# andvg3/LipVQ-VAE

Hardware: AMD Instinct MI355X
Metric: actions tokenized/sec (encode+quantize) at B=4096 T=128 K=1024, 1/2/4/8 GPU (higher is better)
Workload: dtype f32

## Files before the change

lipvq-vae_amd/csrc/lipvq_fused.hip:

```cpp
#include <string.h>
#include <atomic>

#include "lipvq_mlp.h"
#include "lipvq_screen.h"

#define FUSED_WAVES 8
#define FUSED_THREADS (FUSED_WAVES * 64)
#define FUSED_HIST_MAX 2048
#define LQ_RING8_TC 1
#define LQ_RING8_NB 3
#define LQ_RING13_NB 3
constexpr int fused_ring_tc(int S) { return (S <= 2) ? 4 : (S <= 4) ? 2 : (S == 8) ? LQ_RING8_TC : 1; }
constexpr int fused_ring_nb(int S) { return (S <= 4) ? 4 : (S == 8) ? LQ_RING8_NB : LQ_RING13_NB; }
#define LQ_COARSE_TC_WIDE 2
constexpr int fused_ring_tc_coarse(int S) { return S == 8 ? LQ_COARSE_TC_WIDE * fused_ring_tc(S) : fused_ring_tc(S); }

struct Gelu2 {
    lq_v2f x, t, u, s;
    __device__ __forceinline__ void stage0(float a, float b) {
        x = (lq_v2f){a, b};
        t = x * x;
        u = lq_fma2(t, lq_bc2(0.11111111111111111111f), lq_bc2(-1.0f));
        s = lq_fma2(lq_bc2(0.00012666420661844313f), u, lq_bc2(-0.00043783686123788357f));
        s = lq_fma2(s, u, lq_bc2(0.0008924771682359278f));
// ... 45 lines not shown
template <int S, bool FAST>
__host__ __device__ static bool fused_hist_fits(int A, int K) {
    return K <= FUSED_HIST_MAX && fused_lds_bytes_nohist<S, FAST>(A) + (size_t)K * 4 <= (size_t)160 * 1024;
}
template <int S, bool FAST>
static size_t fused_lds_bytes(int A, int K) {
    return fused_lds_bytes_nohist<S, FAST>(A) + (fused_hist_fits<S, FAST>(A, K) ? (size_t)K * 4 : 0);
}

struct TokArgs {
    const float* x;
    const float* packed;
    const unsigned char* packed16;
    const unsigned char* prep;
    const float* cb;
    int64_t* idx;
    float* zq;
    unsigned long long* usage;
    float* ze_out;
    int* amb_count;
    int* amb_list;
    const float* w2q;
    float* pre0;
    float* pre1;
    float* pre2;
    int64_t N;
    int A, D, K;
    float gamma;
    int coarse;
    int inplace;
    int defer_ze;
    int nt_ze;
    int ze_ring;
};

template <int S, bool FAST, bool TRAIN, int WAVES, bool COARSE = false, bool VQ = false>
__device__ __forceinline__ void tokenize_body(const TokArgs& a) {
    static_assert(!(FAST && TRAIN), "training uses the parity arithmetic");
    static_assert(!VQ || !FAST, "the ReLU instance: parity arithmetic");
    constexpr int THREADS = WAVES * 64;
    constexpr int TCF = COARSE ? fused_ring_tc_coarse(S) : fused_ring_tc(S), NBF = fused_ring_nb(S);
    using RingCfg = ScreenCfg<S, TCF, COARSE>;
    constexpr size_t SLAB_STRIDE = ScreenCfg<S, fused_ring_tc(S), false>::STAGE_BYTES;
    constexpr int T0 = 2, T1 = 4, T2 = (S + 1) / 2;
    constexpr int S1 = 16 * T0, S2 = 16 * T1;
    constexpr bool STREAM2 = !FAST && S >= LQ_STREAM2_MIN_S;
    static_assert(!FAST || (S % 2 == 0 && S <= 8), "fast mode: D in {32, 64, 128}");
    extern __shared__ __attribute__((aligned(16))) unsigned char lds[];
#ifdef LQ_STAMPS
    const long long st_top = __builtin_amdgcn_s_memtime();
    const long long st_top_rt = (long long)__builtin_amdgcn_s_memrealtime();
#endif

    const PackedLayout PL = packed_layout(a.A, 32 * T0, 32 * T1, 16 * S);
    const PrepLayout L = prep_layout(a.K, a.D);
    const int S0 = PL.S0;
    const int S0q = (S0 + 3) / 4;
    const int S0h = (a.A + 15) / 16;
    float* w_P0 = reinterpret_cast<float*>(lds);
    float* w_B0 = w_P0 + (FAST ? T0 * S0h * 256 : T0 * S0q * 256);
    float* w_P1 = w_B0 + 32 * T0;
    float* w_B1 = w_P1 + (FAST ? T1 * (2 * T0) * 256 : T1 * (S1 / 4) * 256);
    float* w_P2 = w_B1 + 32 * T1;
    float* w_B2 = w_P2 + (FAST ? T2 * (2 * T1) * 256 : STREAM2 ? 0 : T2 * (S2 / 4) * 256);
    float* w_mu = w_B2 + 32 * T2;
    unsigned char* stage0 = reinterpret_cast<unsigned char*>(w_mu + 16 * S);
    constexpr size_t RING_OWN = (size_t)NBF * RingCfg::STAGE_BYTES + 1024, RING_FINE = lq_ring_bytes<S, fused_ring_tc(S), NBF>();
    constexpr size_t STAGES_BYTES = RING_OWN > RING_FINE ? RING_OWN : RING_FINE;
    static_assert(STAGES_BYTES >= (size_t)WAVES * LQ_DECIDE_BYTES, "the decision's per-wave transposes live in the stage ring");
    constexpr size_t WSLICE = (STAGES_BYTES >= (size_t)WAVES * 8192) ? 8192 : LQ_DECIDE_BYTES;
    static_assert(LQ_DECIDE_BYTES >= 4096 && WSLICE >= LQ_DECIDE_BYTES, "a slice holds the transposes and four staged KiB");
    unsigned* hist = reinterpret_cast<unsigned*>(stage0 + ((STAGES_BYTES + 63) & ~(size_t)63));
    const bool use_hist = a.usage && fused_hist_fits<S, FAST>(a.A, a.K);

    const int tid = threadIdx.x, lane = tid & 63;
    const int wave = __builtin_amdgcn_readfirstlane(tid >> 6);
    const int ln = lane & 31, h = lane >> 5;

    const unsigned* hdr = reinterpret_cast<const unsigned*>(a.prep);
    const unsigned char* tiles = a.prep + (COARSE ? L.o_tiles_hi : L.o_tiles);
    const size_t tile_bytes = COARSE ? L.tile_bytes_hi : L.tile_bytes;
    const int sz = lq_scale_exp(1.0f + __uint_as_float(hdr[4]));
    const float fz = lq_pow2f(sz);
    const float fown = lq_pow2f(sz + (int)hdr[3]);
    const float tiny2 = (float)(16 * S) * lq_pow2f(-10 - 2 * sz);
    const int64_t nblk = (a.N + WAVES * 32 - 1) / (WAVES * 32);
    constexpr int XPF = 8;
    const bool x_pref = !FAST && a.A <= 2 * XPF;
    float xq[XPF];
    constexpr int LANE_W_MIN_S = 8;
    auto load_x = [&](int64_t blk_, float (&out)[XPF]) {
        int64_t r_ = (blk_ * WAVES + wave) * 32 + ln;
        r_ = r_ < a.N ? r_ : a.N - 1;
        const int64_t last = a.N * a.A - 1;
        int h_x = h;
        if constexpr (S >= LANE_W_MIN_S) asm volatile("" : "+v"(h_x));
#pragma unroll
        for (int q = 0; q < XPF; ++q) {
            const int k = 2 * q + h_x;
            int64_t i_ = r_ * a.A + k;
            i_ = i_ < last ? i_ : last;
            const float v = a.x[i_];
            out[q] = (k < a.A) ? v : 0.0f;
        }
// ... 89 lines not shown
#define LQ_STAMP(i) do { const long long t_ = __builtin_amdgcn_s_memtime(); st_acc[i] += t_ - st_prev; st_prev = t_; } while (0)
#else
#define LQ_STAMP(i) do { } while (0)
#endif
    constexpr bool DEFER_GATHER = !FAST;
    int pend_k = 0;
    bool pend_ok = false;
    int64_t pend_row0 = 0;
    bool have_pend = false;
    int64_t ze_shift = 0;
    auto store_ze_tile = [&](const int64_t row, const int t, const f32x16& acc) {
            {
                float lo8[8], hi8[8];
#pragma unroll
                for (int j = 0; j < 8; ++j) {
                    const auto sw = __builtin_amdgcn_permlane32_swap(__float_as_uint(acc[j]), __float_as_uint(acc[8 + j]), false, false);
                    lo8[j] = __uint_as_float(sw[0]);
                    hi8[j] = __uint_as_float(sw[1]);
                }
                if (row < a.N && 2 * t + h < S) {
                    float4* dst = reinterpret_cast<float4*>(a.ze_out + (size_t)(row - ze_shift) * a.D + 32 * t + 16 * h);
                    typedef float lq_f4v __attribute__((ext_vector_type(4)));
#pragma unroll
                    for (int q = 0; q < 4; ++q)
                        if (S > 4 || TRAIN || a.nt_ze) __builtin_nontemporal_store((lq_f4v){lo8[2 * q], hi8[2 * q], lo8[2 * q + 1], hi8[2 * q + 1]}, reinterpret_cast<lq_f4v*>(dst) + q);
                        else reinterpret_cast<lq_f4v*>(dst)[q] = (lq_f4v){lo8[2 * q], hi8[2 * q], lo8[2 * q + 1], hi8[2 * q + 1]};
                }
            }
    };
    for (int64_t blk = blockIdx.x; blk < nblk; blk += gridDim.x) {
#ifdef LQ_STAMPS
        st_prev = __builtin_amdgcn_s_memtime();
#endif
        ze_shift = a.ze_ring ? (blk - (int64_t)blockIdx.x) * (WAVES * 32) : 0;
        f16x8 ah[S], al[S];
        constexpr bool DEFER_ZE = S <= 4 && !TRAIN;
        f32x16 zdef;
        float row_n2, row_a2, row_fz, row_fown;
      auto encode = [&]() {
        int lane_w = lane;
        if constexpr (S >= LANE_W_MIN_S) asm volatile("" : "+v"(lane_w));
        const int h_w = lane_w >> 5;
        const int64_t row0 = (blk * WAVES + wave) * 32;
        const int64_t row = row0 + ln;
        const int64_t rowc = row < a.N ? row : a.N - 1;
        float n2 = 0.0f, a2lo = 0.0f, amax = 0.0f;
        float zt[VQ ? T2 : 1][16];
        auto finish_tile = [&](const int t, f32x16& acc) {
            if constexpr (TRAIN) lq_tile_store16(a.pre2, a.D, row, row < a.N, t, h, acc, a.D, true);
          if constexpr (VQ) {
#pragma unroll
            for (int r = 0; r < 16; ++r) {
                if (2 * t + (r >> 3) >= S) { zt[t][r] = 0.0f; continue; }
                const float zv = acc[r] > 0.0f ? acc[r] : 0.0f;
                acc[r] = zv;
                const float v = zv - w_mu[32 * t + 2 * r + h_w];
                zt[t][r] = v;
                n2 = lq_fma(v, v, n2);
                amax = fmaxf(amax, lq_abs(v));
            }
          } else {
            if constexpr (!FAST) {
                lq_v2f chk = lq_bc2(0.0f);
#pragma unroll
                for (int r = 0; r < 16; r += 2) chk = lq_nonfinite_acc2((lq_v2f){acc[r], acc[r + 1]}, chk);
                if (__builtin_amdgcn_ballot_w64(!(chk.x == 0.0f && chk.y == 0.0f)) != 0ull) {
#pragma unroll
                    for (int r = 0; r < 16; ++r) acc[r] = lq_sigmoid(acc[r]);
                } else {
#pragma unroll
                    for (int r = 0; r < 16; r += 2) {
                        if (2 * t + (r >> 3) >= S) continue;
                        const lq_v2f z2 = lq_sigmoid2_finite((lq_v2f){acc[r], acc[r + 1]});
                        acc[r] = z2.x; acc[r + 1] = z2.y;
                    }
                }
            }
#pragma unroll
            for (int r = 0; r < 16; ++r) {
                if (2 * t + (r >> 3) >= S) continue;
                const float zv = FAST ? __builtin_amdgcn_rcpf(1.0f + __builtin_amdgcn_exp2f(acc[r] * -1.44269504088896341f)) : acc[r];
                acc[r] = zv;
                const float v = zv - w_mu[32 * t + 2 * r + h_w];
                n2 = lq_fma(v, v, n2);
                const float vs = v * fz;
                const _Float16 vh = (_Float16)vs;
                const float rs = vs - (float)vh;
                ah[2 * t + (r >> 3)][r & 7] = vh;
                al[2 * t + (r >> 3)][r & 7] = (_Float16)rs;
                if constexpr (COARSE) a2lo = lq_fma(rs, rs, a2lo);
            }
          }
            if (a.ze_out) {
                if (DEFER_ZE && a.defer_ze && t == T2 - 1) zdef = acc;
                else store_ze_tile(row, t, acc);
            }
        };

        if constexpr (!FAST) {
            auto gelu_fixup = [&](f32x16& out, const f32x16& pre) {
                float mx = 0.0f;
#pragma unroll
                for (int r = 0; r < 16; r += 2) asm("v_max3_f32 %0, %1, |%2|, |%3|" : "=v"(mx) : "v"(mx), "v"(pre[r]), "v"(pre[r + 1]));
                if (__builtin_amdgcn_ballot_w64(!(mx * mx < 18.0f)) != 0ull) {
#pragma unroll
                    for (int r = 0; r < 16; ++r)
                        if (!(pre[r] * pre[r] < 18.0f)) out[r] = lq_gelu_tail(pre[r]);
                }
            };
            auto bias16 = [&](const float* wb, int t) {
                f32x16 b;
                const float4* p4 = reinterpret_cast<const float4*>(wb + (2 * t + h) * 16);
#pragma unroll
                for (int q = 0; q < 4; ++q) { const float4 v = p4[q]; b[4 * q] = v.x; b[4 * q + 1] = v.y; b[4 * q + 2] = v.z; b[4 * q + 3] = v.w; }
                return b;
            };
            f32x16 h0[T0];
            constexpr int NTRIP = (16 * S + 63) / 64;
            constexpr int GP = (STAGES_BYTES >= (size_t)WAVES * 8192) ? 8 : 4;
            constexpr int NROUND = NTRIP * (8 / GP);
            unsigned char* gstage = stage0 + (size_t)wave * WSLICE;
            const bool gnow = DEFER_GATHER && have_pend && a.zq;
            if (gnow) lq_gather_dma<GP>(gstage, a.cb, pend_k, pend_ok, pend_row0, a.N, a.D, lane, 0, 0);
            {
#pragma unroll
                for (int t = 0; t < T0; ++t) h0[t] = bias16(w_B0, t);
// ... 256 lines not shown
                    if (2 * t + (r >> 3) >= S) continue;
                    const float vs = zt[t][r] * fzr;
                    const _Float16 vh = (_Float16)vs;
                    const float rs = vs - (float)vh;
                    ah[2 * t + (r >> 3)][r & 7] = vh;
                    al[2 * t + (r >> 3)][r & 7] = (_Float16)rs;
                    if constexpr (COARSE) a2lo = lq_fma(rs, rs, a2lo);
                }
        }
        if constexpr (COARSE) a2lo += __shfl_xor(a2lo, 32, 64);
        row_a2 = a2lo;
      };
        encode();
        float frow[16];
        if constexpr (VQ) lq_row_factors(row_fown, lane, frow);
        else {
#pragma unroll
            for (int r = 0; r < 16; ++r) frow[r] = fown;
        }
        float m1[16], m2[16];
        int k1[16];
#pragma unroll
        for (int r = 0; r < 16; ++r) { m1[r] = INFINITY; m2[r] = INFINITY; k1[r] = 0; }
        LQ_STAMP(3);
        if (x_pref) load_x(blk + gridDim.x < nblk ? blk + gridDim.x : blk, xq);
        constexpr bool PACKF = S <= 4 || S > 8 || COARSE;
        const float zn = COARSE ? lq_coarse_zn(row_a2, row_n2, row_fz, row_fown, __uint_as_float(hdr[5])) : 0.0f;
        float znr[16];
        if constexpr (COARSE) lq_row_factors(zn, lane, znr);
        else {
#pragma unroll
            for (int r = 0; r < 16; ++r) znr[r] = 0.0f;
        }
        const bool have_def = DEFER_ZE && a.defer_ze && a.ze_out != nullptr;
        auto deferred_ze = [&]() { store_ze_tile((blk * WAVES + wave) * 32 + ln, T2 - 1, zdef); };
        lq_screen_core<S, THREADS, TCF, NBF, PACKF, COARSE, 4, decltype(deferred_ze)>(ah, al, tiles, L.ntiles, stage0, tid, frow, znr, m1, m2, k1, have_def, deferred_ze);
        LQ_STAMP(4);
        const unsigned keep_mask = PACKF ? ~((1u << lq_pack_bits(L.ntiles)) - 1u) : 0xffffffffu;
        unsigned char* scratch = stage0 + (size_t)wave * WSLICE;
        const int64_t row0 = (blk * WAVES + wave) * 32;
        const int64_t row = row0 + ln;
        int my_k;
        LqDecision dec;
        bool certified = lq_screen_decide<PACKF, COARSE>(m1, m2, k1, scratch, hdr, row_n2, row_fown, a.gamma, a.K, a.D, lane,
                                                         my_k, dec, PACKF ? lq_pow2f(lq_pack_bits(L.ntiles) - 23) : 0.0f, keep_mask,
                                                         zn, tiles, tile_bytes, ScreenCfg<S, TCF, COARSE>::FRAG_BYTES);
        const bool row_sane = VQ || row_n2 >= tiny2;
        certified = certified && row_sane;
        if (!COARSE && a.inplace)
            certified = lq_screen_decide_inplace<PACKF, 2 * S, VQ ? LIPVQ_DIST_SQSUM : LIPVQ_DIST_NORM>(
                dec, certified, row_sane, my_k, row0 - ze_shift, row < a.N, a.amb_count, a.ze_out, a.cb, a.K, lane, keep_mask, scratch);
        else
            lq_screen_emit<PACKF>(dec, certified, row_sane, my_k, row, row < a.N, a.amb_count, a.amb_list, a.N, a.K, lane, keep_mask, scratch);
        if (h == 0 && row < a.N && certified) {
            a.idx[row] = (int64_t)my_k;
            if (use_hist) atomicAdd(&hist[my_k], 1u);
        }
        if (a.usage && !use_hist) lq_usage_add(a.usage, my_k, h == 0 && row < a.N && certified);
        if (DEFER_GATHER) { pend_k = my_k; pend_ok = certified; pend_row0 = row0; }
        else if (a.zq) lq_screen_gather(a.cb, a.zq, my_k, certified, row0, a.N, a.D, lane);
        if (DEFER_GATHER) have_pend = true;
        LQ_STAMP(5);
        LQ_STAMP(6);
    }
    if (DEFER_GATHER && have_pend && a.zq) lq_screen_gather(a.cb, a.zq, pend_k, pend_ok, pend_row0, a.N, a.D, lane);
#ifdef LQ_STAMPS
    if (lane == 0) {
        long long* dbg = LqWorkspace::from_lists(a.amb_list, a.N).stamps() + ((size_t)blockIdx.x * WAVES + wave) * 16;
        for (int i = 0; i < 7; ++i) dbg[i] = st_acc[i];
        dbg[7] = 0;
        dbg[8] = __builtin_amdgcn_s_memtime() - st_begin;
        dbg[9] = st_begin;
        dbg[10] = st_begin - st_top;
        dbg[11] = (long long)__builtin_amdgcn_s_memrealtime();
        dbg[12] = st_top_rt;
    }
#endif
    lq_ws_publish(a.amb_count);
    if (use_hist) {
        for (int i = tid; i < a.K; i += THREADS) {
            const unsigned c = hist[i];
            if (c) atomicAdd(&a.usage[i], (unsigned long long)c);
        }
    }
}

template <int S, bool FAST, bool TRAIN = false, bool COARSE = false, bool VQ = false>
__global__ __launch_bounds__(FUSED_THREADS) void tokenize_kernel(TokArgs a) {
    tokenize_body<S, FAST, TRAIN, FUSED_WAVES, COARSE, VQ>(a);
}
template <int S, bool FAST, bool TRAIN, bool COARSE = false>
__global__ __launch_bounds__(256) __attribute__((amdgpu_waves_per_eu(1, 1))) void tokenize_kernel_w4(TokArgs a) {
    tokenize_body<S, FAST, TRAIN, 4, COARSE>(a);
}

__global__ void mlp3_pack_f16_kernel(const float* __restrict__ W0, const float* __restrict__ W1, const float* __restrict__ W2,
                                     _Float16* __restrict__ out, int A, int J0, int J1, int D) {
    const int S0h = (A + 15) / 16, S1h = J0 / 16, S2h = J1 / 16;
    const int T0 = J0 / 32, T1 = J1 / 32, T2 = (D + 31) / 32;
    const size_t n0 = (size_t)T0 * S0h * 512, n1 = (size_t)T1 * S1h * 512, n2 = (size_t)T2 * S2h * 512;
    size_t g = (size_t)blockIdx.x * blockDim.x + threadIdx.x;
    if (g >= n0 + n1 + n2) return;
    const float* W;
    int K, J, Sh;
    size_t e = g;
    if (e < n0) { W = W0; K = A; J = J0; Sh = S0h; }
    else if (e < n0 + n1) { e -= n0; W = W1; K = J0; J = J1; Sh = S1h; }
    else { e -= n0 + n1; W = W2; K = J1; J = D; Sh = S2h; }
    const int j = (int)(e & 7), lane = (int)((e >> 3) & 63);
    const size_t ts = e >> 9;
    const int s = (int)(ts % Sh), t = (int)(ts / Sh);
    const int f = 32 * t + feat_of_tile_row(lane & 31);
    const int k = 16 * s + 2 * j + (lane >> 5);
    out[g] = (_Float16)((f < J && k < K) ? W[(size_t)f * K + k] : 0.0f);
}

extern "C" size_t lipvq_mlp3_packed_f16_bytes(int A, int J0, int J1, int D) {
    if (A <= 0 || J0 <= 0 || J1 <= 0 || D <= 0 || (J0 & 31) || (J1 & 31)) return 0;
    const size_t S0h = (A + 15) / 16, T2 = (D + 31) / 32;
    return ((size_t)(J0 / 32) * S0h + (size_t)(J1 / 32) * (J0 / 16) + T2 * (J1 / 16)) * 512 * sizeof(_Float16);
}

extern "C" int lipvq_mlp3_pack_f16_f32(const float* W0, const float* W1, const float* W2, void* packed16, int A, int J0,
                                       int J1, int D, void* stream) {
    if (!W0 || !W1 || !W2 || !packed16) return fail(LIPVQ_EINVAL, "mlp3_pack_f16: null pointer");
    const size_t bytes = lipvq_mlp3_packed_f16_bytes(A, J0, J1, D);
// ... 2 lines not shown
    hipLaunchKernelGGL(mlp3_pack_f16_kernel, dim3((unsigned)((n + 255) / 256)), dim3(256), 0, (hipStream_t)stream, W0, W1, W2,
                       (_Float16*)packed16, A, J0, J1, D);
    return check_launch("mlp3_pack_f16");
}

extern "C" int lipvq_tokenize_supported(int A, int J0, int J1, int D, int K) {
    return (A > 0 && A <= 64 && J0 == 64 && J1 == 128 && K > 0 && (D == 32 || D == 64 || D == 128 || D == 208)) ? 1 : 0;
}

extern "C" int lipvq_tokenize_fast_supported(int A, int J0, int J1, int D, int K) {
    return (lipvq_tokenize_supported(A, J0, J1, D, K) && D != 208) ? 1 : 0;
}

#define LQ_DEFAULT_DEFER_ZE 0
struct LqSchedule { int defer_ze, nt_ze; };
static std::atomic<int> g_tuned[64];
static LqSchedule lq_schedule(int ring) {
    LqSchedule sc{LQ_DEFAULT_DEFER_ZE, ring ? 0 : 1};
    int dev = 0;
    if (hipGetDevice(&dev) == hipSuccess && dev >= 0 && dev < 64) {
        const int t = g_tuned[dev].load(std::memory_order_relaxed);
        if (t) { sc.defer_ze = (t - 1) & 1; sc.nt_ze = ((t - 1) >> 1) & 1; }
    }
    if (const char* e = lq_knob("tok_defer_ze")) sc.defer_ze = e[0] != '0';
    if (const char* e = lq_knob("tok_nt_ze")) sc.nt_ze = e[0] != '0';
    return sc;
}

static int lq_inplace(bool have_ze, int coarse, int K) {
    const char* e = lq_knob("tok_inplace");
    return (have_ze && !coarse && K <= LQ_LISTS_ALL_K && !(e && e[0] == '0')) ? 1 : 0;
}
static int lq_ze_ring(bool caller_wants_ze, int inplace) { return (!caller_wants_ze && inplace) ? 1 : 0; }

static int tok_waves(int64_t N) {
    const char* e = lq_knob("tok_shape");
    if (e && !strcmp(e, "w8rg1")) return 8;
    if (e && !strcmp(e, "w4rg1")) return 4;
    return N <= 4 * 32 * 256 ? 4 : 8;
}

__global__ void w2q_pack_kernel(const float* __restrict__ P2, float* __restrict__ out, int T2, int S2) {
    const size_t i = (size_t)blockIdx.x * blockDim.x + threadIdx.x;
    if (i >= (size_t)T2 * (S2 / 4) * 256) return;
    const int q = (int)(i & 3), l = (int)((i >> 2) & 63), sq = (int)((i >> 8) % (S2 / 4)), t = (int)((i >> 8) / (S2 / 4));
    out[i] = P2[((size_t)t * S2 + 4 * sq + q) * 64 + l];
}

template <int S, bool FAST, bool TRAIN, int WAVES, bool COARSE, bool VQ>
static int launch_tokenize_as(const TokArgs& a, hipStream_t st) {
    static_assert(WAVES == 8 || !VQ, "the plain VQVAE's instances have 8 waves");
    static LqLdsReserve reserved;
    const size_t lds = fused_lds_bytes<S, FAST>(a.A, a.K);
    if (lds > 160 * 1024) return fail(LIPVQ_EUNSUPPORTED, "tokenize: %zu B of LDS needed", lds);
    void (*kfn)(TokArgs);
    if constexpr (WAVES == 4) kfn = tokenize_kernel_w4<S, FAST, TRAIN, COARSE>;
    else kfn = tokenize_kernel<S, FAST, TRAIN, COARSE, VQ>;
    if (int rc = lipvq_reserve_lds(reserved, (const void*)kfn, lds, "tokenize")) return rc;
    if (a.w2q) {
        const PackedLayout PL = packed_layout(a.A, 64, 128, a.D);
        const size_t n = LqWorkspace::w2q_floats(a.D);
        hipLaunchKernelGGL(w2q_pack_kernel, dim3((unsigned)((n + 255) / 256)), dim3(256), 0, st, a.packed + PL.oP2,
                           LqWorkspace::from_lists(a.amb_list, a.N).w2q(), PL.T2, PL.S2);
    }
    const int64_t unit = (int64_t)WAVES * 32;
    const int64_t nblk = (a.N + unit - 1) / unit;
    const int64_t cap = 256;
    hipLaunchKernelGGL(kfn, dim3((unsigned)(nblk < cap ? nblk : cap)), dim3(WAVES * 64), lds, st, a);
    return check_launch("tokenize");
}

enum { TOK_TRAIN, TOK_FAST, TOK_PARITY, TOK_VQ };
template <int S, int MODE>
static int launch_tokenize(const TokArgs& a, hipStream_t st) {
    if constexpr (MODE == TOK_TRAIN) {
        return a.coarse ? launch_tokenize_as<S, false, true, 8, true, false>(a, st) : launch_tokenize_as<S, false, true, 8, false, false>(a, st);
    } else if constexpr (MODE == TOK_FAST) {
        if constexpr (S <= 8) return launch_tokenize_as<S, true, false, 8, false, false>(a, st);
        else return LIPVQ_EUNSUPPORTED;
    } else if constexpr (MODE == TOK_PARITY) {
        const int waves = tok_waves(a.N);
        if constexpr (S >= 8) {
            if (a.coarse && waves == 4) return launch_tokenize_as<S, false, false, 4, true, false>(a, st);
        }
        if (a.coarse) return launch_tokenize_as<S, false, false, 8, true, false>(a, st);
        if (waves == 4) return launch_tokenize_as<S, false, false, 4, false, false>(a, st);
        return launch_tokenize_as<S, false, false, 8, false, false>(a, st);
    } else {
        if (a.pre0) return a.coarse ? launch_tokenize_as<S, false, true, 8, true, true>(a, st) : launch_tokenize_as<S, false, true, 8, false, true>(a, st);
        return a.coarse ? launch_tokenize_as<S, false, false, 8, true, true>(a, st) : launch_tokenize_as<S, false, false, 8, false, true>(a, st);
    }
}

extern "C" int lipvq_tokenize_workspace_init(void* workspace, void* stream) {
    if (!workspace) return fail(LIPVQ_EINVAL, "tokenize_workspace_init: null pointer");
    hipError_t e = hipMemsetAsync(workspace, 0, LqWorkspace::kHeaderBytes, (hipStream_t)stream);
    if (e != hipSuccess) return fail(LIPVQ_EHIP, "tokenize_workspace_init: %s", hipGetErrorString(e));
    return LIPVQ_OK;
}

extern "C" size_t lipvq_tokenize_workspace_bytes(int64_t N, int D) { return (N <= 0 || D <= 0) ? 0 : LqWorkspace::tokenize_bytes(N, D); }

static int tokenize_run(const char* who, bool vq, const float* x, const float* packed, const void* packed16, const float* const* raw6,
                        const float* codebook, const void* prep, int64_t* idx, float* zq, int64_t* usage, float* ze_out,
                        float* pre0, float* pre1, float* pre2, void* workspace, int64_t N, int A, int J0, int J1, int D, int K,
                        void* stream) {
    if (N < 0) return fail(LIPVQ_EINVAL, "%s: N < 0", who);
    if (N == 0) return LIPVQ_OK;
    if (!x || !packed || !codebook || !prep || !idx || !workspace || (vq ? !ze_out : !raw6)) return fail(LIPVQ_EINVAL, "%s: null pointer", who);
    for (int i = 0; !vq && i < 6; ++i)
        if (!raw6[i]) return fail(LIPVQ_EINVAL, "%s: raw encoder weight %d is null", who, i);
    if (!lipvq_tokenize_supported(A, J0, J1, D, K))
        return fail(LIPVQ_EUNSUPPORTED, "%s: unsupported shape A=%d J0=%d J1=%d D=%d K=%d", who, A, J0, J1, D, K);
    if (N > 2147483647LL) return fail(LIPVQ_EUNSUPPORTED, "%s: N too large", who);
    if ((((uintptr_t)codebook | (uintptr_t)zq | (uintptr_t)ze_out | (uintptr_t)workspace | (uintptr_t)packed16 | (uintptr_t)pre0 |
          (uintptr_t)pre1 | (uintptr_t)pre2) & 15) != 0)
        return fail(LIPVQ_EINVAL, "%s: codebook, zq, ze_out, workspace, packed16 and pre0..2 must be 16-byte aligned", who);
    if (packed16 && !lipvq_tokenize_fast_supported(A, J0, J1, D, K))
        return fail(LIPVQ_EUNSUPPORTED, "%s: D=%d has no fast instance (32, 64, 128)", who, D);
    hipStream_t st = (hipStream_t)stream;
    const LqWorkspace ws{(unsigned char*)workspace, N, D};
    const LqOut out{idx, zq, usage};
    const int coarse = !packed16 ? lq_screen_coarse(lq_screen_S(D), K) : 0;
    int64_t ze_rows = packed16 ? 131072 : INT64_MAX;
    if (const char* ev = lq_knob("tok_ze_rows")) ze_rows = atoll(ev);
    float* ze_buf = (ze_out || !(coarse || N <= ze_rows)) ? ze_out : ws.ze_scratch();
    TokArgs a{};
    a.x = x;
    a.packed = packed;
    a.packed16 = (const unsigned char*)packed16;
    a.prep = (const unsigned char*)prep;
    a.cb = codebook;
    a.idx = idx;
    a.zq = zq;
    a.usage = (unsigned long long*)usage;
    a.ze_out = ze_buf;
    a.amb_count = ws.live();
    a.amb_list = ws.row_list();
    a.w2q = LqWorkspace::w2q_floats(D) ? ws.w2q() : nullptr;
    a.pre0 = pre0;
    a.pre1 = pre1;
    a.pre2 = pre2;
    a.N = N;
    a.A = A;
    a.D = D;
    a.K = K;
    a.gamma = LIPVQ_SCREEN_GAMMA;
    a.coarse = coarse;
    a.inplace = lq_inplace(ze_buf != nullptr, coarse, K);
    a.ze_ring = lq_ze_ring(ze_out != nullptr, a.inplace);
    const LqSchedule sc = lq_schedule(a.ze_ring);
    a.defer_ze = sc.defer_ze;
    a.nt_ze = sc.nt_ze;
    int rc = LIPVQ_OK;
    lq_dispatch<TOK_TRAIN, TOK_FAST, TOK_PARITY, TOK_VQ>(vq ? TOK_VQ : pre0 ? TOK_TRAIN : packed16 ? TOK_FAST : TOK_PARITY, [&](auto mode) {
        lq_dispatch<32, 64, 128, 208>(D, [&](auto d) { rc = launch_tokenize<(d() + 15) / 16, mode()>(a, st); });
    });
    if (!rc && !a.inplace) {
        if (ze_buf) rc = lipvq_launch_rows(ze_buf, 0, codebook, out, ws, K, st, vq ? LIPVQ_DIST_SQSUM : LIPVQ_DIST_NORM);
        else rc = lipvq_launch_rows_encode(x, raw6, A, codebook, out, ws, K, st);
    }
    if (rc) (void)hipMemsetAsync(ws.header(), 0, LqWorkspace::kHeaderBytes, st);
    return rc;
}

extern "C" int lipvq_tokenize_f32(const float* x, const float* packed, const float* const* raw6, const float* codebook,
                                  const void* prep, int64_t* idx, float* zq, int64_t* usage, float* ze_out,
                                  void* workspace, int64_t N, int A, int J0, int J1, int D, int K, void* stream) {
    return tokenize_run("tokenize", false, x, packed, nullptr, raw6, codebook, prep, idx, zq, usage, ze_out, nullptr, nullptr, nullptr,
                        workspace, N, A, J0, J1, D, K, stream);
}

extern "C" int lipvq_tokenize_tune_f32(const float* x, const float* packed, const float* const* raw6, const float* codebook,
                                       const void* prep, int64_t* idx, float* zq, int64_t* usage, float* ze_out, void* workspace,
                                       int64_t N, int A, int J0, int J1, int D, int K, void* stream, int launches, int* choice,
                                       float* ms4) {
    hipStream_t st = (hipStream_t)stream;
    hipStreamCaptureStatus cs = hipStreamCaptureStatusNone;
    if (hipStreamIsCapturing(st, &cs) == hipSuccess && cs != hipStreamCaptureStatusNone)
        return fail(LIPVQ_EINVAL, "tokenize_tune: the stream is capturing (the tuner synchronises)");
    if (launches < 1) return fail(LIPVQ_EINVAL, "tokenize_tune: launches < 1");
    if (lq_screen_S(D) > 4) {
        if (choice) *choice = -1;
        if (ms4) for (int c = 0; c < 4; ++c) ms4[c] = 0.0f;
        return LIPVQ_OK;
    }
    int dev = 0;
    if (hipGetDevice(&dev) != hipSuccess || dev < 0 || dev >= 64) return fail(LIPVQ_EINVAL, "tokenize_tune: device index");
    hipEvent_t e0, e1;
    if (hipEventCreate(&e0) != hipSuccess || hipEventCreate(&e1) != hipSuccess) return fail(LIPVQ_EHIP, "tokenize_tune: hipEventCreate");
    const int before = g_tuned[dev].load(std::memory_order_relaxed);
    float best[4] = {INFINITY, INFINITY, INFINITY, INFINITY};
    int rc = LIPVQ_OK;
    auto run = [&](int n) {
        for (int i = 0; i < n && !rc; ++i)
            rc = lipvq_tokenize_f32(x, packed, raw6, codebook, prep, idx, zq, usage, ze_out, workspace, N, A, J0, J1, D, K, stream);
    };
    run(launches);
    for (int round = 0; round < 2 && !rc; ++round)
        for (int c = 0; c < 4 && !rc; ++c) {
            g_tuned[dev].store(1 + c, std::memory_order_relaxed);
            run((launches + 1) / 2);
            (void)hipEventRecord(e0, st);
            run(launches);
            (void)hipEventRecord(e1, st);
            if (hipEventSynchronize(e1) != hipSuccess) rc = fail(LIPVQ_EHIP, "tokenize_tune: hipEventSynchronize");
            float ms = 0.0f;
            if (!rc && hipEventElapsedTime(&ms, e0, e1) == hipSuccess && ms / launches < best[c]) best[c] = ms / launches;
        }
    (void)hipEventDestroy(e0);
    (void)hipEventDestroy(e1);
    if (rc) { g_tuned[dev].store(before, std::memory_order_relaxed); return rc; }
    const int ring = lq_ze_ring(ze_out != nullptr, lq_inplace(true, lq_screen_coarse(lq_screen_S(D), K), K));
    const int dflt = LQ_DEFAULT_DEFER_ZE | ((ring ? 0 : 1) << 1);
    int win = dflt;
    for (int c = 0; c < 4; ++c) if (best[c] < 0.995f * best[dflt] && best[c] < best[win]) win = c;
    g_tuned[dev].store(1 + win, std::memory_order_relaxed);
    if (choice) *choice = win;
    if (ms4) for (int c = 0; c < 4; ++c) ms4[c] = best[c];
    return LIPVQ_OK;
}

extern "C" int lipvq_tokenize_train_f32(const float* x, const float* packed, const float* const* raw6, const float* codebook,
                                        const void* prep, int64_t* idx, float* zq, int64_t* usage, float* ze_out, float* pre0,
                                        float* pre1, float* pre2, void* workspace, int64_t N, int A, int J0, int J1, int D, int K,
                                        void* stream) {
    if (!ze_out || !pre0 || !pre1 || !pre2) return fail(LIPVQ_EINVAL, "tokenize_train: z_e and the three pre-activation buffers are required");
    return tokenize_run("tokenize_train", false, x, packed, nullptr, raw6, codebook, prep, idx, zq, usage, ze_out, pre0, pre1, pre2,
                        workspace, N, A, J0, J1, D, K, stream);
}

// ... 24 lines not shown
```

lipvq-vae_amd/csrc/lipvq_screen.h:

```cpp
#ifndef LIPVQ_SCREEN_H_
#define LIPVQ_SCREEN_H_
#include <hip/hip_fp16.h>

#include <type_traits>

#include "lipvq_common.h"

typedef _Float16 f16x8 __attribute__((ext_vector_type(8)));

#define LIPVQ_SCREEN_GAMMA 3.814697265625e-06f
#define SCREEN_WAVES 8

struct PrepLayout {
    int S, Dpad, Kpad, ntiles;
    size_t o_hdr, o_mu, o_tiles, tile_bytes, total;
    size_t o_tiles_hi, tile_bytes_hi;
};

#define LIPVQ_SCREEN_GAMMA_WIDE 1.52587890625e-05f
#define LQ_SCREEN_NARROW_MAX_S 13

__host__ __device__ static inline int lq_screen_S(int D) {
    const int s = (D + 15) / 16;
    return D <= 0 ? 0 : s <= 2 ? 2 : s <= 4 ? 4 : s <= 8 ? 8 : s <= 13 ? 13 : s <= 16 ? 16 : s <= 24 ? 24 : s <= 32 ? 32 : 0;
// ... 78 lines not shown
}

template <int S, bool PACK, bool COARSE = false>
__device__ __forceinline__ void lq_track_after_mfma(int j, const f32x16& acc, float e2, float en, const float (&frow)[16],
                                                    const float (&znr)[16], int id, unsigned keep_mask, float (&m1)[16],
                                                    float (&m2)[16], int (&k1)[16]) {
    constexpr int NM = COARSE ? S : 3 * S;
    const int lo = (16 * j) / NM, hi = (16 * (j + 1)) / NM;
#pragma unroll
    for (int r = 0; r < 16; ++r)
        if (r >= lo && r < hi) {
            const float v = COARSE ? acc[r] : lq_fma(e2, frow[r], acc[r]);
            lq_track_one<PACK>(v, id, keep_mask, m1[r], m2[r], k1[r]);
        }
}

template <int N>
__device__ __forceinline__ void lq_wait_vmcnt() {
    static_assert(N >= 0 && N < 64, "vmcnt immediate");
    asm volatile("s_waitcnt vmcnt(%0)" ::"n"(N) : "memory");
}
template <int S, int TC_, int NB>
constexpr size_t lq_ring_bytes() { return (size_t)NB * ScreenCfg<S, TC_>::STAGE_BYTES + 1024; }

__host__ __device__ static inline int lq_pack_bits(int ntiles) { int b = 1; while ((1 << b) < ntiles) ++b; return b; }

struct LqNoDeferred { __device__ __forceinline__ void operator()() const {} };
template <int S, int NT, int TC_ = screen_default_tc(S), int NB = 4, bool PACK = false, bool COARSE = false, int NDEF = 0,
          typename DEFERRED = LqNoDeferred>
__device__ __forceinline__ void lq_screen_core(const f16x8 (&ah)[S], const f16x8 (&al)[S],
                                               const unsigned char* __restrict__ tiles, int ntiles,
                                               unsigned char* stage0, int tid, const float (&frow)[16], const float (&znr)[16],
                                               float (&m1)[16], float (&m2)[16], int (&k1)[16],
                                               bool have_def = false, DEFERRED deferred = DEFERRED()) {
    using C = ScreenCfg<S, TC_, COARSE>;
    static_assert(NB >= 3 && NB <= 4, "ring of 3 or 4 stage buffers");
    constexpr int NW = NT / 64;
    constexpr int CHUNKS = (C::STAGE_BYTES + 1023) / 1024;
    constexpr int CPW = (CHUNKS + NW - 1) / NW;
    constexpr int PD = NB - 1;
    constexpr int NSTEP = C::TC * S;
    constexpr int MID = (C::TC >= 2) ? (C::TC / 2) * S : S / 2;
    constexpr int FR = 2;
    constexpr int FD = FR - 1;
    constexpr int PERIOD = ((C::TC & 1) || (NSTEP % FR)) ? 2 : 1;
    static_assert(C::STAGE_BYTES >= 1024 && C::STAGE_BYTES % 16 == 0, "stage copies are whole KiB pieces");
    static_assert(NSTEP - FD >= MID, "next-stage fragments are read after the hand-over");
    static_assert(CPW * PD < 64, "vmcnt immediate");
    const int lane = tid & 63, ln = lane & 31;
    const int wave = __builtin_amdgcn_readfirstlane(tid >> 6);
    const int nstage = ntiles / C::TC;
    unsigned char* dummy = stage0 + (size_t)NB * C::STAGE_BYTES;
    typedef __attribute__((address_space(3))) void* lds_ptr_t;
    typedef const __attribute__((address_space(1))) void* glb_ptr_t;
    auto stage_dma = [&](int st, int buf) {
        const bool real = st < nstage;
        const unsigned char* src = tiles + (real ? (size_t)st * C::STAGE_BYTES : (size_t)0);
        unsigned char* dst = stage0 + (size_t)buf * C::STAGE_BYTES;
#pragma unroll
        for (int j = 0; j < CPW; ++j) {
            int chunk = wave + j * NW;
            chunk = chunk < CHUNKS ? chunk : CHUNKS - 1;
            int off = chunk * 1024;
            off = off + 1024 <= C::STAGE_BYTES ? off : C::STAGE_BYTES - 1024;
            unsigned char* d = real ? dst + off : dummy;
            __builtin_amdgcn_global_load_lds((glb_ptr_t)(src + off + lane * 16), (lds_ptr_t)d, 16, 0, 0);
        }
    };
    auto frag = [&](const unsigned char* tb, int s, int hl) {
        return COARSE ? *reinterpret_cast<const f16x8*>(tb + ((size_t)s * 64 + lane) * 16)
                      : *reinterpret_cast<const f16x8*>(tb + (((size_t)s * 2 + hl) * 64 + lane) * 16);
    };
    lq_wg_barrier();
#pragma unroll
    for (int p = 0; p < PD; ++p) stage_dma(p, p);
    static_assert((PD - 1) * CPW + NDEF < 64, "vmcnt immediate");
    if (NDEF > 0 && have_def) {
        deferred();
        lq_wait_vmcnt<(PD - 1) * CPW + NDEF>();
    } else {
        lq_wait_vmcnt<(PD - 1) * CPW>();
    }
    lq_wg_barrier();

    f32x16 accA, accB;
#pragma unroll
    for (int r = 0; r < 16; ++r) accB[r] = INFINITY;
    float e2A = 0.0f, e2B = 0.0f;
    int codeA = 0, codeB = 0;
    const unsigned keep_mask = PACK ? ~((1u << lq_pack_bits(ntiles)) - 1u) : 0xffffffffu;
    f16x8 fh[FR], fl[FR];
    float e2q[2] = {0.0f, 0.0f};
    float enq[2] = {0.0f, 0.0f};
    float enA = 0.0f, enB = 0.0f;
#pragma unroll
    for (int g = 0; g < FD; ++g) {
        fh[g] = frag(stage0, g, 0);
        if constexpr (!COARSE) fl[g] = frag(stage0, g, 1);
    }
    e2q[0] = reinterpret_cast<const float*>(stage0 + C::FRAG_BYTES)[ln];
    if constexpr (COARSE) enq[0] = reinterpret_cast<const float*>(stage0 + C::FRAG_BYTES + 128)[ln];
    static_assert(FD <= S, "prologue reads stay in tile 0");
    int buf = 0;
    auto do_stage = [&](auto POS, int st) {
        constexpr int par = (decltype(POS)::value * C::TC) & 1;
        constexpr int so = (decltype(POS)::value * NSTEP) % FR;
        const unsigned char* sb = stage0 + (size_t)buf * C::STAGE_BYTES;
        int nbuf = buf + 1; nbuf = nbuf == NB ? 0 : nbuf;
        const unsigned char* nsb = stage0 + (size_t)nbuf * C::STAGE_BYTES;
#pragma unroll
        for (int g = 0; g < NSTEP; ++g) {
            const int c = g / S, s = g % S;
            if (g == MID) {
                if (NDEF > 0 && have_def && st == 0) lq_wait_vmcnt<(PD >= 2 ? (PD - 2) * CPW : 0) + (PD >= 2 ? NDEF : 0)>();
                else lq_wait_vmcnt<(PD >= 2 ? (PD - 2) * CPW : 0)>();
                lq_wg_barrier();
                int b = buf + PD; b = b >= NB ? b - NB : b;
                stage_dma(st + PD, b);
            }
            f32x16& acc = (((c + par) & 1) == 0) ? accA : accB;
            const f32x16& prev = (((c + par) & 1) == 0) ? accB : accA;
            const float e2_prev = (((c + par) & 1) == 0) ? e2B : e2A;
            const float en_prev = (((c + par) & 1) == 0) ? enB : enA;
            const int code_prev = (((c + par) & 1) == 0) ? codeB : codeA;
            if (s == 0) {
                const float e2c = e2q[(c + par) & 1];
                const float enc = enq[(c + par) & 1];
#pragma unroll
                for (int r = 0; r < 16; ++r) acc[r] = COARSE ? lq_fma(-znr[r], enc, e2c * frow[r]) : 0.0f;
                int code = PACK ? (st * C::TC + c) : (st * C::TC + c) * 32 + ln;
                if constexpr (PACK) asm volatile("" : "+v"(code));
                if (((c + par) & 1) == 0) { e2A = e2c; enA = enc; codeA = code; } else { e2B = e2c; enB = enc; codeB = code; }
            }
            const f16x8 bh = fh[(g + so) % FR];
            f16x8 bl = bh;
            if constexpr (!COARSE) bl = fl[(g + so) % FR];
            auto read_ahead = [&]() {
                const int g1 = g + FD;
                const unsigned char* base = (g1 < NSTEP) ? sb : nsb;
                const int gg = (g1 < NSTEP) ? g1 : g1 - NSTEP;
                const unsigned char* tb = base + (size_t)(gg / S) * C::TILE_BYTES;
                fh[(g1 + so) % FR] = frag(tb, gg % S, 0);
                if constexpr (!COARSE) fl[(g1 + so) % FR] = frag(tb, gg % S, 1);
                if (gg % S == 0) {
                    e2q[(g1 / S + par) & 1] = reinterpret_cast<const float*>(tb + C::FRAG_BYTES)[ln];
                    if constexpr (COARSE) enq[(g1 / S + par) & 1] = reinterpret_cast<const float*>(tb + C::FRAG_BYTES + 128)[ln];
                }
// ... 326 lines not shown
        if constexpr (DIST == LIPVQ_DIST_NORM) {
            float a = 0.0f;
#pragma unroll
            for (int i = 0; i < DCH; ++i) { const float d = zv[i] - c[8 * i + j]; a = lq_fma(d, d, a); }
            s = __shfl(a, 8 * g, 64);
#pragma unroll
            for (int l = 1; l < 8; ++l) s = s + __shfl(a, 8 * g + l, 64);
            s = lq_sqrt(s);
        } else {
            float acc[4] = {0.f, 0.f, 0.f, 0.f};
#pragma unroll
            for (int i = 0; i < DCH; ++i) {
                const int q = (i < (DCH / 4) * 4) ? (i & 3) : 0;
                const float d = zv[i] - c[8 * i + j];
                acc[q] = acc[q] + d * d;
            }
            const float vl = ((acc[0] + acc[1]) + acc[2]) + acc[3];
            s = __shfl(vl, 8 * g, 64);
#pragma unroll
            for (int l = 1; l < 8; ++l) s = s + __shfl(vl, 8 * g + l, 64);
        }
        const float v = (live && s == s) ? s : INFINITY;
        const int kk = live ? code : 0x7fffffff;
        LQ_TAKE_MIN(best_v, best_k, v, kk);
    }
    LQ_WAVE_MIN(best_v, best_k, 8);
    if (best_k < 0 || best_k >= K) {
        const int fb = scanning ? __builtin_ctz(lm_eff) : LQ_SLOT_FIRST(cl, n0);
        best_k = (fb >= 0 && fb < K) ? fb : 0;
    }
    return best_k;
}

template <bool PACK, int DCH, int DIST>
__device__ __forceinline__ bool lq_screen_decide_inplace(const LqDecision& dec, bool certified, bool lists_ok, int& my_k, int64_t row0,
                                                         bool row_valid, int* __restrict__ amb_count, const float* __restrict__ z,
                                                         const float* __restrict__ cb, int K, int lane, unsigned keep_mask,
                                                         unsigned char* wave_lds) {
    const bool need = row_valid && !certified;
    if (__builtin_amdgcn_ballot_w64(need) == 0ull) return certified;
    const int ln = lane & 31, h = lane >> 5;
    unsigned long long lm = __builtin_amdgcn_ballot_w64(h == 0 && need);
    if (lane == __builtin_ctzll(lm)) (void)lq_ws_reserve(amb_count, __builtin_popcountll(lm));
    int head;
    unsigned mask;
    int codes[LQ_CAND_MAX];
    lq_emit_candidates<PACK>(dec, lists_ok, K, lane, keep_mask, wave_lds, head, mask, codes);
    __builtin_amdgcn_wave_barrier();
    int* parts = reinterpret_cast<int*>(wave_lds);
    static_assert(LQ_CAND_MAX == 6 && 32 * 16 * 4 <= LQ_DECIDE_BYTES, "a part is {n, mask, six codes}");
    if (need) {
        typedef int lq_i4 __attribute__((ext_vector_type(4)));
        lq_i4* out4 = reinterpret_cast<lq_i4*>(parts + ln * 16 + 8 * h);
        out4[0] = lq_i4{head, (int)mask, codes[0], codes[1]};
        out4[1] = lq_i4{codes[2], codes[3], codes[4], codes[5]};
    }
    __builtin_amdgcn_s_waitcnt(0xC07F);
    __builtin_amdgcn_wave_barrier();
    constexpr int D = DCH * 8;
    while (lm) {
        const int r = __builtin_ctzll(lm);
        lm &= lm - 1ull;
        const float* zr = z + (size_t)(row0 + r) * D;
        const int bk = lq_lists_row<DCH, DIST>([&](int f) { return __hip_atomic_load(zr + f, __ATOMIC_RELAXED, __HIP_MEMORY_SCOPE_AGENT); },
                                               cb, K, parts + r * 16, lane, true);
        if (ln == r) { my_k = bk; certified = true; }
    }
    __builtin_amdgcn_wave_barrier();
    return certified;
}

struct LqGatherTrip { float4 val[8]; };
__device__ __forceinline__ void lq_gather_load(LqGatherTrip& g, const float* __restrict__ cb, int my_k, bool row_ok, int64_t row0,
                                               int64_t N, int D, int lane, int trip) {
    const int nvec = D / 4;
    const int v = 16 * trip + (lane & 15);
    const int vc = v < nvec ? v : nvec - 1;
#pragma unroll
    for (int p = 0; p < 8; ++p) {
        const int src_lane = 4 * p + (lane >> 4);
        const int kk = __shfl(my_k, src_lane, 64);
        const bool ok = (__shfl((int)row_ok, src_lane, 64) != 0) && (row0 + src_lane < N);
        g.val[p] = reinterpret_cast<const float4*>(cb + (size_t)(ok ? kk : 0) * D)[vc];
    }
}
__device__ __forceinline__ void lq_gather_store(const LqGatherTrip& g, float* __restrict__ zq, bool row_ok, int64_t row0, int64_t N,
                                                int D, int lane, int trip) {
    const int nvec = D / 4;
    const int v = 16 * trip + (lane & 15);
#pragma unroll
    for (int p = 0; p < 8; ++p) {
        const int src_lane = 4 * p + (lane >> 4);
        const bool ok = (__shfl((int)row_ok, src_lane, 64) != 0) && (row0 + src_lane < N) && (v < nvec);
        if (ok) reinterpret_cast<float4*>(zq + (size_t)(row0 + src_lane) * D)[v] = g.val[p];
    }
}
template <int NP>
__device__ __forceinline__ void lq_gather_dma(unsigned char* wave_stage, const float* __restrict__ cb, int my_k, bool row_ok,
// ... 62 lines not shown
```

Baseline: 1.350 billion.

## Keep z_e in registers for in-place decisions instead of a global ring

When the caller does not want z_e and the in-place decision path is used for narrow parity instances, the encoder output tiles are now held in registers and copied into LDS, one row at a time, only for ambiguous rows. Before, they were written to a global ring buffer and read back with atomic loads. This removes the z_e global stores and the deferred-store bookkeeping. The cost is extra register pressure and LDS traffic. The change also makes the deferred-store vmcnt accounting per wave and skips the autotune sweep when keepz applies.

```diff
diff --git a/lipvq-vae_amd/csrc/lipvq_fused.hip b/lipvq-vae_amd/csrc/lipvq_fused.hip
--- a/lipvq-vae_amd/csrc/lipvq_fused.hip
+++ b/lipvq-vae_amd/csrc/lipvq_fused.hip
@@ -101,12 +101,14 @@
     int defer_ze;
     int nt_ze;
     int ze_ring;
+    int keepz;
 };
 
-template <int S, bool FAST, bool TRAIN, int WAVES, bool COARSE = false, bool VQ = false>
+template <int S, bool FAST, bool TRAIN, int WAVES, bool COARSE = false, bool VQ = false, bool KEEPZ = false>
 __device__ __forceinline__ void tokenize_body(const TokArgs& a) {
     static_assert(!(FAST && TRAIN), "training uses the parity arithmetic");
     static_assert(!VQ || !FAST, "the ReLU instance: parity arithmetic");
+    static_assert(!KEEPZ || (S <= 4 && !FAST && !TRAIN && !COARSE && !VQ), "z_e kept in registers: the narrow parity instances, decided in place");
     constexpr int THREADS = WAVES * 64;
     constexpr int TCF = COARSE ? fused_ring_tc_coarse(S) : fused_ring_tc(S), NBF = fused_ring_nb(S);
     using RingCfg = ScreenCfg<S, TCF, COARSE>;
@@ -139,6 +141,7 @@
     static_assert(STAGES_BYTES >= (size_t)WAVES * LQ_DECIDE_BYTES, "the decision's per-wave transposes live in the stage ring");
     constexpr size_t WSLICE = (STAGES_BYTES >= (size_t)WAVES * 8192) ? 8192 : LQ_DECIDE_BYTES;
     static_assert(LQ_DECIDE_BYTES >= 4096 && WSLICE >= LQ_DECIDE_BYTES, "a slice holds the transposes and four staged KiB");
+    static_assert(!KEEPZ || WSLICE >= LQ_DECIDE_BYTES + 64 * S, "KEEPZ: one z_e row behind the decision scratch");
     unsigned* hist = reinterpret_cast<unsigned*>(stage0 + ((STAGES_BYTES + 63) & ~(size_t)63));
     const bool use_hist = a.usage && fused_hist_fits<S, FAST>(a.A, a.K);
 
@@ -294,10 +297,11 @@
 #ifdef LQ_STAMPS
         st_prev = __builtin_amdgcn_s_memtime();
 #endif
-        ze_shift = a.ze_ring ? (blk - (int64_t)blockIdx.x) * (WAVES * 32) : 0;
+        ze_shift = (!KEEPZ && a.ze_ring) ? (blk - (int64_t)blockIdx.x) * (WAVES * 32) : 0;
         f16x8 ah[S], al[S];
-        constexpr bool DEFER_ZE = S <= 4 && !TRAIN;
+        constexpr bool DEFER_ZE = S <= 4 && !TRAIN && !KEEPZ;
         f32x16 zdef;
+        f32x16 zkeep[KEEPZ ? T2 : 1];
         float row_n2, row_a2, row_fz, row_fown;
       auto encode = [&]() {
         int lane_w = lane;
@@ -353,7 +357,9 @@
                 if constexpr (COARSE) a2lo = lq_fma(rs, rs, a2lo);
             }
           }
-            if (a.ze_out) {
+            if constexpr (KEEPZ) {
+                zkeep[t] = acc;
+            } else if (a.ze_out) {
                 if (DEFER_ZE && a.defer_ze && t == T2 - 1) zdef = acc;
                 else store_ze_tile(row, t, acc);
             }
@@ -676,9 +682,14 @@
 #pragma unroll
             for (int r = 0; r < 16; ++r) znr[r] = 0.0f;
         }
-        const bool have_def = DEFER_ZE && a.defer_ze && a.ze_out != nullptr;
-        auto deferred_ze = [&]() { store_ze_tile((blk * WAVES + wave) * 32 + ln, T2 - 1, zdef); };
-        lq_screen_core<S, THREADS, TCF, NBF, PACKF, COARSE, 4, decltype(deferred_ze)>(ah, al, tiles, L.ntiles, stage0, tid, frow, znr, m1, m2, k1, have_def, deferred_ze);
+        if constexpr (KEEPZ) {
+            lq_screen_core<S, THREADS, TCF, NBF, PACKF, COARSE>(ah, al, tiles, L.ntiles, stage0, tid, frow, znr, m1, m2, k1);
+        } else {
+            const bool have_def = DEFER_ZE && a.defer_ze && a.ze_out != nullptr;
+            const bool wave_def = __builtin_amdgcn_ballot_w64((blk * WAVES + wave) * 32 + ln < a.N) != 0ull;
+            auto deferred_ze = [&]() { store_ze_tile((blk * WAVES + wave) * 32 + ln, T2 - 1, zdef); };
+            lq_screen_core<S, THREADS, TCF, NBF, PACKF, COARSE, 4, decltype(deferred_ze)>(ah, al, tiles, L.ntiles, stage0, tid, frow, znr, m1, m2, k1, have_def, deferred_ze, wave_def);
+        }
         LQ_STAMP(4);
         const unsigned keep_mask = PACKF ? ~((1u << lq_pack_bits(L.ntiles)) - 1u) : 0xffffffffu;
         unsigned char* scratch = stage0 + (size_t)wave * WSLICE;
@@ -691,7 +702,10 @@
                                                          zn, tiles, tile_bytes, ScreenCfg<S, TCF, COARSE>::FRAG_BYTES);
         const bool row_sane = VQ || row_n2 >= tiny2;
         certified = certified && row_sane;
-        if (!COARSE && a.inplace)
+        if constexpr (KEEPZ)
+            certified = lq_screen_decide_inplace<PACKF, 2 * S, LIPVQ_DIST_NORM, T2>(
+                dec, certified, row_sane, my_k, row0, row < a.N, a.amb_count, nullptr, a.cb, a.K, lane, keep_mask, scratch, zkeep);
+        else if (!COARSE && a.inplace)
             certified = lq_screen_decide_inplace<PACKF, 2 * S, VQ ? LIPVQ_DIST_SQSUM : LIPVQ_DIST_NORM>(
                 dec, certified, row_sane, my_k, row0 - ze_shift, row < a.N, a.amb_count, a.ze_out, a.cb, a.K, lane, keep_mask, scratch);
         else
@@ -729,13 +743,13 @@
     }
 }
 
-template <int S, bool FAST, bool TRAIN = false, bool COARSE = false, bool VQ = false>
+template <int S, bool FAST, bool TRAIN = false, bool COARSE = false, bool VQ = false, bool KEEPZ = false>
 __global__ __launch_bounds__(FUSED_THREADS) void tokenize_kernel(TokArgs a) {
-    tokenize_body<S, FAST, TRAIN, FUSED_WAVES, COARSE, VQ>(a);
-}
-template <int S, bool FAST, bool TRAIN, bool COARSE = false>
+    tokenize_body<S, FAST, TRAIN, FUSED_WAVES, COARSE, VQ, KEEPZ>(a);
+}
+template <int S, bool FAST, bool TRAIN, bool COARSE = false, bool KEEPZ = false>
 __global__ __launch_bounds__(256) __attribute__((amdgpu_waves_per_eu(1, 1))) void tokenize_kernel_w4(TokArgs a) {
-    tokenize_body<S, FAST, TRAIN, 4, COARSE>(a);
+    tokenize_body<S, FAST, TRAIN, 4, COARSE, false, KEEPZ>(a);
 }
 
 __global__ void mlp3_pack_f16_kernel(const float* __restrict__ W0, const float* __restrict__ W1, const float* __restrict__ W2,
@@ -804,6 +818,7 @@
     return (have_ze && !coarse && K <= LQ_LISTS_ALL_K && !(e && e[0] == '0')) ? 1 : 0;
 }
 static int lq_ze_ring(bool caller_wants_ze, int inplace) { return (!caller_wants_ze && inplace) ? 1 : 0; }
+static int lq_keepz(int ring, bool parity, int D) { return (ring && parity && lq_screen_S(D) <= 4) ? 1 : 0; }
 
 static int tok_waves(int64_t N) {
     const char* e = lq_knob("tok_shape");
@@ -819,15 +834,15 @@
     out[i] = P2[((size_t)t * S2 + 4 * sq + q) * 64 + l];
 }
 
-template <int S, bool FAST, bool TRAIN, int WAVES, bool COARSE, bool VQ>
+template <int S, bool FAST, bool TRAIN, int WAVES, bool COARSE, bool VQ, bool KEEPZ = false>
 static int launch_tokenize_as(const TokArgs& a, hipStream_t st) {
     static_assert(WAVES == 8 || !VQ, "the plain VQVAE's instances have 8 waves");
     static LqLdsReserve reserved;
     const size_t lds = fused_lds_bytes<S, FAST>(a.A, a.K);
     if (lds > 160 * 1024) return fail(LIPVQ_EUNSUPPORTED, "tokenize: %zu B of LDS needed", lds);
     void (*kfn)(TokArgs);
-    if constexpr (WAVES == 4) kfn = tokenize_kernel_w4<S, FAST, TRAIN, COARSE>;
-    else kfn = tokenize_kernel<S, FAST, TRAIN, COARSE, VQ>;
+    if constexpr (WAVES == 4) kfn = tokenize_kernel_w4<S, FAST, TRAIN, COARSE, KEEPZ>;
+    else kfn = tokenize_kernel<S, FAST, TRAIN, COARSE, VQ, KEEPZ>;
     if (int rc = lipvq_reserve_lds(reserved, (const void*)kfn, lds, "tokenize")) return rc;
     if (a.w2q) {
         const PackedLayout PL = packed_layout(a.A, 64, 128, a.D);
@@ -856,6 +871,10 @@
             if (a.coarse && waves == 4) return launch_tokenize_as<S, false, false, 4, true, false>(a, st);
         }
         if (a.coarse) return launch_tokenize_as<S, false, false, 8, true, false>(a, st);
+        if constexpr (S <= 4) {
+            if (a.keepz) return waves == 4 ? launch_tokenize_as<S, false, false, 4, false, false, true>(a, st)
+                                           : launch_tokenize_as<S, false, false, 8, false, false, true>(a, st);
+        }
         if (waves == 4) return launch_tokenize_as<S, false, false, 4, false, false>(a, st);
         return launch_tokenize_as<S, false, false, 8, false, false>(a, st);
     } else {
@@ -921,9 +940,15 @@
     a.coarse = coarse;
     a.inplace = lq_inplace(ze_buf != nullptr, coarse, K);
     a.ze_ring = lq_ze_ring(ze_out != nullptr, a.inplace);
-    const LqSchedule sc = lq_schedule(a.ze_ring);
-    a.defer_ze = sc.defer_ze;
-    a.nt_ze = sc.nt_ze;
+    a.keepz = lq_keepz(a.ze_ring, !vq && !pre0 && !packed16, D);
+    if (a.keepz) {
+        a.ze_out = nullptr;
+        a.ze_ring = 0;
+    } else {
+        const LqSchedule sc = lq_schedule(a.ze_ring);
+        a.defer_ze = sc.defer_ze;
+        a.nt_ze = sc.nt_ze;
+    }
     int rc = LIPVQ_OK;
     lq_dispatch<TOK_TRAIN, TOK_FAST, TOK_PARITY, TOK_VQ>(vq ? TOK_VQ : pre0 ? TOK_TRAIN : packed16 ? TOK_FAST : TOK_PARITY, [&](auto mode) {
         lq_dispatch<32, 64, 128, 208>(D, [&](auto d) { rc = launch_tokenize<(d() + 15) / 16, mode()>(a, st); });
@@ -969,6 +994,20 @@
             rc = lipvq_tokenize_f32(x, packed, raw6, codebook, prep, idx, zq, usage, ze_out, workspace, N, A, J0, J1, D, K, stream);
     };
     run(launches);
+    if (lq_keepz(lq_ze_ring(ze_out != nullptr, lq_inplace(true, lq_screen_coarse(lq_screen_S(D), K), K)), true, D)) {
+        float ms = 0.0f;
+        (void)hipEventRecord(e0, st);
+        run(launches);
+        (void)hipEventRecord(e1, st);
+        if (!rc && hipEventSynchronize(e1) != hipSuccess) rc = fail(LIPVQ_EHIP, "tokenize_tune: hipEventSynchronize");
+        if (!rc && hipEventElapsedTime(&ms, e0, e1) != hipSuccess) rc = fail(LIPVQ_EHIP, "tokenize_tune: hipEventElapsedTime");
+        (void)hipEventDestroy(e0);
+        (void)hipEventDestroy(e1);
+        if (rc) return rc;
+        if (choice) *choice = LQ_DEFAULT_DEFER_ZE | (1 << 1);
+        if (ms4) for (int c = 0; c < 4; ++c) ms4[c] = ms / launches;
+        return LIPVQ_OK;
+    }
     for (int round = 0; round < 2 && !rc; ++round)
         for (int c = 0; c < 4 && !rc; ++c) {
             g_tuned[dev].store(1 + c, std::memory_order_relaxed);
diff --git a/lipvq-vae_amd/csrc/lipvq_screen.h b/lipvq-vae_amd/csrc/lipvq_screen.h
--- a/lipvq-vae_amd/csrc/lipvq_screen.h
+++ b/lipvq-vae_amd/csrc/lipvq_screen.h
@@ -134,7 +134,7 @@
                                                const unsigned char* __restrict__ tiles, int ntiles,
                                                unsigned char* stage0, int tid, const float (&frow)[16], const float (&znr)[16],
                                                float (&m1)[16], float (&m2)[16], int (&k1)[16],
-                                               bool have_def = false, DEFERRED deferred = DEFERRED()) {
+                                               bool have_def = false, DEFERRED deferred = DEFERRED(), bool wave_def = true) {
     using C = ScreenCfg<S, TC_, COARSE>;
     static_assert(NB >= 3 && NB <= 4, "ring of 3 or 4 stage buffers");
     constexpr int NW = NT / 64;
@@ -177,8 +177,9 @@
 #pragma unroll
     for (int p = 0; p < PD; ++p) stage_dma(p, p);
     static_assert((PD - 1) * CPW + NDEF < 64, "vmcnt immediate");
-    if (NDEF > 0 && have_def) {
-        deferred();
+    const bool count_def = NDEF > 0 && have_def && wave_def;
+    if (NDEF > 0 && have_def) deferred();
+    if (count_def) {
         lq_wait_vmcnt<(PD - 1) * CPW + NDEF>();
     } else {
         lq_wait_vmcnt<(PD - 1) * CPW>();
@@ -214,7 +215,7 @@
         for (int g = 0; g < NSTEP; ++g) {
             const int c = g / S, s = g % S;
             if (g == MID) {
-                if (NDEF > 0 && have_def && st == 0) lq_wait_vmcnt<(PD >= 2 ? (PD - 2) * CPW : 0) + (PD >= 2 ? NDEF : 0)>();
+                if (count_def && st == 0) lq_wait_vmcnt<(PD >= 2 ? (PD - 2) * CPW : 0) + (PD >= 2 ? NDEF : 0)>();
                 else lq_wait_vmcnt<(PD >= 2 ? (PD - 2) * CPW : 0)>();
                 lq_wg_barrier();
                 int b = buf + PD; b = b >= NB ? b - NB : b;
@@ -607,11 +608,12 @@
     return best_k;
 }
 
-template <bool PACK, int DCH, int DIST>
+template <bool PACK, int DCH, int DIST, int NKEEP = 0>
 __device__ __forceinline__ bool lq_screen_decide_inplace(const LqDecision& dec, bool certified, bool lists_ok, int& my_k, int64_t row0,
                                                          bool row_valid, int* __restrict__ amb_count, const float* __restrict__ z,
                                                          const float* __restrict__ cb, int K, int lane, unsigned keep_mask,
-                                                         unsigned char* wave_lds) {
+                                                         unsigned char* wave_lds ,
+                                                         const f32x16* zkeep = nullptr) {
     const bool need = row_valid && !certified;
     if (__builtin_amdgcn_ballot_w64(need) == 0ull) return certified;
     const int ln = lane & 31, h = lane >> 5;
@@ -636,9 +638,25 @@
     while (lm) {
         const int r = __builtin_ctzll(lm);
         lm &= lm - 1ull;
-        const float* zr = z + (size_t)(row0 + r) * D;
-        const int bk = lq_lists_row<DCH, DIST>([&](int f) { return __hip_atomic_load(zr + f, __ATOMIC_RELAXED, __HIP_MEMORY_SCOPE_AGENT); },
-                                               cb, K, parts + r * 16, lane, true);
+        int bk;
+        if constexpr (NKEEP > 0) {
+            static_assert(NKEEP * 32 == D, "the kept tiles are the row");
+            float* zrow = reinterpret_cast<float*>(wave_lds + LQ_DECIDE_BYTES);
+            if (ln == r) {
+#pragma unroll
+                for (int t = 0; t < NKEEP; ++t)
+#pragma unroll
+                    for (int q = 0; q < 16; ++q) zrow[32 * t + 2 * q + h] = zkeep[t][q];
+            }
+            __builtin_amdgcn_s_waitcnt(0xC07F);
+            __builtin_amdgcn_wave_barrier();
+            bk = lq_lists_row<DCH, DIST>([&](int f) { return zrow[f]; }, cb, K, parts + r * 16, lane, true);
+            __builtin_amdgcn_wave_barrier();
+        } else {
+            const float* zr = z + (size_t)(row0 + r) * D;
+            bk = lq_lists_row<DCH, DIST>([&](int f) { return __hip_atomic_load(zr + f, __ATOMIC_RELAXED, __HIP_MEMORY_SCOPE_AGENT); },
+                                         cb, K, parts + r * 16, lane, true);
+        }
         if (ln == r) { my_k = bk; certified = true; }
     }
     __builtin_amdgcn_wave_barrier();
```

After: 1.373 billion (median of 6 runs). 1.7% higher.
